# sanweiliti/LEMO

Measured on AMD Instinct MI355X. Metric: fitting-iterations/sec (T=120 frames), higher is better.
Workload: dtype f32; 1 GPU; opt_amass_temp.py temporal fit, one TotalCapture-shaped clip per GPU: B=119 frames (the T=120 clip), SMPL-X-shaped synthetic model V=10475, VPoser decode, smoothness encoder 245x134, marker+contact+prior losses, Adam; frames=119, vertices_per_frame=10475, sequences=1, conv_variant=9, parallelism=seq-shard x1 + 1 all_gather, hip_graph=True

## Files before the change

### lemo_amd/csrc/conv_turn_kernels.hip

```cpp
#include "conv_common.hpp"
#include "conv_f16.hpp"
#include "conv_pair.hpp"
#include "loss_device.hpp"

namespace lemo {

constexpr int TT_TH = 12, TT_TW = 12;
constexpr int TT_INW = TT_TW + 6, TT_INH = TT_TH + 4, TT_NIN = TT_INW * TT_INH;
constexpr int TT_ZW = TT_TW + 4, TT_ZH = TT_TH + 2, TT_NZ = TT_ZW * TT_ZH;
constexpr int TT_DW = TT_TW + 2, TT_DH = TT_TH + 2, TT_ND = TT_DW * TT_DH;
constexpr int TT_DP = 20, TT_NDP = TT_DP * TT_DH;
constexpr int TT_NOUT = TT_TH * TT_TW;
constexpr int TT_PL_IN = TT_NIN * 16, TT_GRP_IN = 2 * TT_PL_IN;
constexpr int TT_PL_D = TT_NDP * 16, TT_GRP_D = 2 * TT_PL_D;
constexpr int TT_D_OFF = 8 * TT_GRP_IN;
constexpr int TT_WMAX_OFF = TT_D_OFF + 8 * TT_GRP_D;
constexpr int TT_SMEM = TT_WMAX_OFF + 4 * 8 * 4;
constexpr int TT_NSLOT = 5;
constexpr int TT_NITEM = 8 * TT_ND * 2, TT_KITEM = (TT_NITEM + 511) / 512;
constexpr int TT_FRAMES = 32;
static_assert(TT_ZW == 16 && TT_NZ == 7 * 32 && TT_INW == 18, "z N-tiles = 2 rows x 16 columns on the input grid of row pitch 18");
static_assert(4 * 2 * TT_NIN <= TT_NSLOT * 512 && TT_NOUT <= 5 * 32, "staging slots / output tiles");
static_assert(8 * 8 * 256 * 4 <= TT_D_OFF && 8 * 6 * 256 * 4 <= TT_D_OFF, "the K-half exchanges fit the dead input planes");
static_assert(8 * TT_NZ * 8 * 4 <= 8 * TT_GRP_D, "the fp32 z tile fits the (not yet written) dpre planes");

__constant__ unsigned short tt_pix[160] = {
    0,   1,   2,   3,   12,  13,  14,  15,  16,  17,  18,  19,  4,   5,   6,   7,   28,  29,  30,  31,  8,   9,   10,  11,
    20,  21,  22,  23,  32,  33,  34,  35,  24,  25,  26,  27,  48,  49,  50,  51,  52,  53,  54,  55,  36,  37,  38,  39,
    56,  57,  58,  59,  40,  41,  42,  43,  44,  45,  46,  47,  68,  69,  70,  71,  60,  61,  62,  63,  72,  73,  74,  75,
    84,  85,  86,  87,  64,  65,  66,  67,  88,  89,  90,  91,  76,  77,  78,  79,  80,  81,  82,  83,  92,  93,  94,  95,
    96,  97,  98,  99,  108, 109, 110, 111, 112, 113, 114, 115, 100, 101, 102, 103, 124, 125, 126, 127, 104, 105, 106, 107,
    116, 117, 118, 119, 128, 129, 130, 131, 120, 121, 122, 123, 256, 257, 258, 259, 260, 261, 262, 263, 132, 133, 134, 135,
    264, 265, 266, 267, 136, 137, 138, 139, 140, 141, 142, 143, 276, 277, 278, 279};

struct TurnArgs {
  const float* in;
  const uint4* wf;
  const uint4* wb;
  const float* bias;
  float* z;
  float* out;
  float* dpre;
  double* acc;
  float winvf, winvb, coef2;
  int H, W, ntx, ntiles;
  FrameLoss fl;
  int nfb;
  unsigned long long* dbg;
};

struct TurnZ { float4 v[8]; int po[2]; bool own[2]; };

template <int NT>
__device__ __forceinline__ void turn_forward(const TurnArgs& a, unsigned char* smem, float* smem_f, float* wmax, int y0, int x0, int g, int ch,
                                             int kh, int lane, int wave, uint4 (&ra)[CP_RA][2], float (&sc)[2], float (&sci)[2],
                                             float4 (&stB)[TT_NSLOT], const int (&dstB)[TT_NSLOT], TurnZ& zs) {
  const int j = lane & 31, h = lane >> 5, T0 = g ? 4 : 0;
  const int H = a.H, W = a.W, Wp = W + 2;
  int li[NT];
#pragma unroll
  for (int nt = 0; nt < NT; ++nt) li[nt] = (2 * (T0 + nt) + (j >> 4) + 1) * TT_INW + cp_lane_col(j) + 1;
  f32x16 acc[NT];
#pragma unroll
  for (int nt = 0; nt < NT; ++nt)
#pragma unroll
    for (int r = 0; r < 16; ++r) acc[nt][r] = 0.f;
  pair_kloop<NT, TT_GRP_IN, TT_PL_IN, TT_INW>(
      acc, ra, a.wf, smem, li, kh, ch, lane,
      [&](int cc, int tap) {
        if (cc != 0) return;
        if (tap == 0) {
          float m = 0.f;
#pragma unroll
          for (int k = 0; k < TT_NSLOT; ++k) m = absmax4(stB[k], m);
          m = wave_max(m);
          if (lane == 0) wmax[8 + wave] = m;
        }
        if (tap == 1) {
          __syncthreads();
          float mm = 0.f;
#pragma unroll
          for (int i = 0; i < 8; ++i) mm = fmaxf(mm, wmax[8 + i]);
          f16_scale_after(mm, sc[0], sc[1], sci[1]);
        }
#pragma unroll
        for (int k = 0; k < TT_NSLOT; ++k) {
          if (2 + (7 * k) / TT_NSLOT != tap) continue;
          uint2 s0, s1;
          split2x4(stB[k], sc[1], s0, s1);
          *reinterpret_cast<uint2*>(smem + 2 * TT_GRP_IN + dstB[k]) = s0;
          *reinterpret_cast<uint2*>(smem + 2 * TT_GRP_IN + dstB[k] + TT_PL_IN) = s1;
        }
      },
      [&](int cc) {
        __syncthreads();
        if (cc == 0) {
          const float f = sc[1] * sci[0];
#pragma unroll
          for (int nt = 0; nt < NT; ++nt)
#pragma unroll
            for (int r = 0; r < 16; ++r) acc[nt][r] *= f;
        }
      });
  {
    const float f = sci[1] * a.winvf;
#pragma unroll
    for (int nt = 0; nt < NT; ++nt)
#pragma unroll
      for (int r = 0; r < 16; ++r) acc[nt][r] *= f;
  }
  typedef PairSplit<NT> S;
  const int KHu = __builtin_amdgcn_readfirstlane(kh);
  int zp[2];
  bool inimg[2];
#pragma unroll
  for (int sl = 0; sl < 2; ++sl) {
    const int t = T0 + (sl == 0 ? KHu : (NT == 4 ? 2 + KHu : 2));
    const int zr = 2 * t + (j >> 4), zc = cp_lane_col(j);
    const int y = y0 - 1 + zr, x = x0 - 2 + zc;
    zp[sl] = zr * TT_ZW + zc;
    inimg[sl] = (unsigned)y < (unsigned)H && (unsigned)x < (unsigned)W;
    zs.own[sl] = inimg[sl] && zr >= 1 && zr <= TT_TH && zc >= 2 && zc <= TT_TW + 1;
    const int yc = y < 0 ? 0 : (y >= H ? H - 1 : y), xc = x < 0 ? 0 : (x >= W ? W - 1 : x);
    zs.po[sl] = (yc + 1) * Wp + (xc + 1);
  }
  float4 eo[S::NQ];
#pragma unroll
  for (int i = 0; i < S::NQ; ++i) {
    const int q = KHu ? S::keep_quad(1, i) : S::keep_quad(0, i);
    eo[i] = ld4(a.bias + ch * 32 + q * 8 + 4 * h);
  }
  float4 v[S::NQ];
  {
    float* red = smem_f + ((g * 2 + ch) * 2) * 2048 + lane * 4;
    if (KHu) pair_exchange<NT, 1>(acc, v, red + 2048, red);
    else pair_exchange<NT, 0>(acc, v, red, red + 2048);
  }
  float* zt = smem_f + TT_D_OFF / 4;
#pragma unroll
  for (int i = 0; i < S::NQ; ++i) {
    const int q = KHu ? S::keep_quad(1, i) : S::keep_quad(0, i);
    const int c0 = ch * 32 + q * 8 + 4 * h;
    float4 r = v[i];
    r.x = lrelu(r.x + eo[i].x); r.y = lrelu(r.y + eo[i].y); r.z = lrelu(r.z + eo[i].z); r.w = lrelu(r.w + eo[i].w);
    if (!(i < 4 ? inimg[0] : inimg[1])) r = make_float4(0.f, 0.f, 0.f, 0.f);
    st4(zt + ((c0 >> 3) * TT_NZ + (i < 4 ? zp[0] : zp[1])) * 8 + (c0 & 7), r);
    zs.v[i] = r;
  }
}

template <bool DBG, int NT>
__device__ __forceinline__ void turn_backward(const TurnArgs& a, unsigned char* smem, float* smem_f, int y0, int x0, int T0, int g, int ch,
                                              int kh, int lane, float smi, uint4 (&ra)[CP_RA][2]) {
  const int j = lane & 31, h = lane >> 5;
  const int Wp = a.W + 2, HWp = (a.H + 2) * Wp;
  int lo[NT], poff[NT];
  bool ok[NT];
#pragma unroll
  for (int nt = 0; nt < NT; ++nt) {
    const int e = tt_pix[(T0 + nt) * 32 + j], p = e & 255, oy = p / TT_TW, ox = p - oy * TT_TW;
    lo[nt] = (oy + 1) * TT_DP + ox + 1;
    const int y = y0 + oy, x = x0 + ox;
    ok[nt] = e < 256 && y < a.H && x < a.W;
    poff[nt] = ((y < a.H ? y : a.H - 1) + 1) * Wp + ((x < a.W ? x : a.W - 1) + 1);
  }
  f32x16 acc[NT];
#pragma unroll
  for (int nt = 0; nt < NT; ++nt)
#pragma unroll
    for (int r = 0; r < 16; ++r) acc[nt][r] = 0.f;
  pair_kloop<NT, TT_GRP_D, TT_PL_D, TT_DP>(acc, ra, a.wb, smem + TT_D_OFF, lo, kh, ch, lane, [](int, int) {}, [](int) {});
  {
    const float f = smi * a.winvb;
#pragma unroll
    for (int nt = 0; nt < NT; ++nt)
#pragma unroll
      for (int r = 0; r < 16; ++r) acc[nt][r] *= f;
  }
  typedef PairSplit<NT> S;
  const int KHu = __builtin_amdgcn_readfirstlane(kh);
  const int poA = KHu ? poff[1] : poff[0], poB = poff[NT - 1];
  const bool okA = KHu ? ok[1] : ok[0], okB = ok[NT - 1];
  float4 eo[S::NQ];
#pragma unroll
  for (int i = 0; i < S::NQ; ++i) {
    const int q = KHu ? S::keep_quad(1, i) : S::keep_quad(0, i);
    const int c0 = ch * 32 + q * 8 + 4 * h;
    eo[i] = ld4(a.in + ((size_t)(c0 >> 3) * HWp + (i < 4 ? poA : poB)) * 8 + (c0 & 7));
  }
  float* red = smem_f + ((g * 2 + ch) * 2) * 1536 + lane * 4;
  float4 v[S::NQ];
  if (KHu) pair_exchange<NT, 1>(acc, v, red + 1536, red);
  else pair_exchange<NT, 0>(acc, v, red, red + 1536);
#pragma unroll
  for (int i = 0; i < S::NQ; ++i) {
    const int q = KHu ? S::keep_quad(1, i) : S::keep_quad(0, i);
    const int c0 = ch * 32 + q * 8 + 4 * h;
    float4 r = v[i];
    r.x *= lrelu_grad_from_out(eo[i].x); r.y *= lrelu_grad_from_out(eo[i].y);
    r.z *= lrelu_grad_from_out(eo[i].z); r.w *= lrelu_grad_from_out(eo[i].w);
    if (i < 4 ? okA : okB) st4(a.out + ((size_t)(c0 >> 3) * HWp + (i < 4 ? poA : poB)) * 8 + (c0 & 7), r);
  }
}

template <bool DBG>
__global__ void __launch_bounds__(512)
conv3x3_turn_kernel(TurnArgs a) {
  const int tid = (int)threadIdx.x, lane = tid & 63, wave = tid >> 6;
  if ((int)blockIdx.x >= a.ntiles) {
    const int b = ((int)blockIdx.x - a.ntiles) * TT_FRAMES + wave * 4 + (lane >> 4);
    vertex_loss_row16(b, lane & 15, a.fl);
    return;
  }
  unsigned long long t_start = 0, t_pro = 0, t_z = 0, t_st = 0, t_pl = 0;
  if (DBG) t_start = __builtin_amdgcn_s_memtime();
  LEMO_DYN_SMEM(smem_f);
  unsigned char* smem = reinterpret_cast<unsigned char*>(smem_f);
  float* wmax = reinterpret_cast<float*>(smem + TT_WMAX_OFF);
  const int ng = wave & 1, ch = (wave >> 1) & 1, kh = wave >> 2;
  const int H = a.H, W = a.W, Wp = W + 2, HWp = (H + 2) * Wp;
  const unsigned in_gstride = (unsigned)HWp * 8u;
  int tile = (int)blockIdx.x;
  {
    const int q = a.ntiles >> 3, r = a.ntiles & 7, xcd = tile & 7, k = tile >> 3;
    tile = (xcd < r ? xcd * (q + 1) : r * (q + 1) + (xcd - r) * q) + k;
  }
  const int ty = tile / a.ntx, tx = tile - ty * a.ntx;
  const int y0 = ty * TT_TH, x0 = tx * TT_TW;
  const int g = __builtin_amdgcn_readfirstlane(ng ^ kh);

  uint4 ra[CP_RA][2];
  pair_preload_a(ra, a.wf, kh, ch, lane);

  unsigned offB[TT_NSLOT];
  int dstB[TT_NSLOT];
#pragma unroll
  for (int k = 0; k < TT_NSLOT; ++k) {
    int c0 = tid + k * 512;
    c0 = c0 < 4 * 2 * TT_NIN ? c0 : 4 * 2 * TT_NIN - 1;
    const int gg = c0 / (2 * TT_NIN), c = c0 - gg * (2 * TT_NIN);
    const int px = c >> 1, half = c & 1;
    const int r = px / TT_INW, col = px - r * TT_INW;
    int gy = y0 - 2 + r, gx = x0 - 3 + col;
    gy = (gy < -1 ? -1 : (gy > H ? H : gy)) + 1;
    gx = (gx < -1 ? -1 : (gx > W ? W : gx)) + 1;
    const int g0 = (gg >> 1) * 4 + (gg & 1);
    offB[k] = (unsigned)g0 * in_gstride + (unsigned)(gy * Wp + gx) * 8u + 4u * half;
    dstB[k] = g0 * TT_GRP_IN + px * 16 + 8 * half;
  }
  float4 stB[TT_NSLOT];
#pragma unroll
  for (int k = 0; k < TT_NSLOT; ++k) stB[k] = ld4(a.in + offB[k]);
  float sc[2] = {1.f, 1.f}, sci[2] = {1.f, 1.f};
  {
    float m = 0.f;
#pragma unroll
    for (int k = 0; k < TT_NSLOT; ++k) m = absmax4(stB[k], m);
    m = wave_max(m);
    if (lane == 0) wmax[wave] = m;
    __syncthreads();
    float mm = 0.f;
#pragma unroll
    for (int i = 0; i < 8; ++i) mm = fmaxf(mm, wmax[i]);
    f16_scale_for(mm, sc[0], sci[0]);
  }
#pragma unroll
  for (int k = 0; k < TT_NSLOT; ++k) {
    uint2 s0, s1;
    split2x4(stB[k], sc[0], s0, s1);
    *reinterpret_cast<uint2*>(smem + dstB[k]) = s0;
    *reinterpret_cast<uint2*>(smem + dstB[k] + TT_PL_IN) = s1;
  }
#pragma unroll
  for (int k = 0; k < TT_NSLOT; ++k) stB[k] = ld4(a.in + 2u * in_gstride + offB[k]);
  __syncthreads();
  if (DBG) t_pro = __builtin_amdgcn_s_memtime();

  TurnZ zs;
  if (g) turn_forward<3>(a, smem, smem_f, wmax, y0, x0, 1, ch, kh, lane, wave, ra, sc, sci, stB, dstB, zs);
  else turn_forward<4>(a, smem, smem_f, wmax, y0, x0, 0, ch, kh, lane, wave, ra, sc, sci, stB, dstB, zs);
  pair_preload_a(ra, a.wb, kh, ch, lane);
  __syncthreads();
  if (DBG) t_z = __builtin_amdgcn_s_memtime();

  const float* zt = smem_f + TT_D_OFF / 4;
  float4 dv[TT_KITEM];
  int dslot[TT_KITEM];
  float sq = 0.f, mloc = 0.f;
#pragma unroll
  for (int k = 0; k < TT_KITEM; ++k) {
    const int it = tid + k * 512, ic = it < TT_NITEM ? it : TT_NITEM - 1;
    const int half = ic & 1, rest = ic >> 1, gq = rest / TT_ND, dp = rest - gq * TT_ND;
    const int dr = dp / TT_DW, dc = dp - dr * TT_DW;
    const int y = y0 - 1 + dr, x = x0 - 1 + dc;
    const bool valid = it < TT_NITEM && (unsigned)y < (unsigned)H && (unsigned)x < (unsigned)W;
    const bool own = valid && dr >= 1 && dr <= TT_TH && dc >= 1 && dc <= TT_TW;
    const bool hasl = x >= 1, hasr = x <= W - 2;
    const float* zc = zt + (gq * TT_NZ + dr * TT_ZW + dc + 1) * 8 + 4 * half;
    const float4 c = ld4(zc), l = ld4(zc - 8), r = ld4(zc + 8);
    float4 gr = make_float4(0.f, 0.f, 0.f, 0.f);
    if (hasl) { gr.x += c.x - l.x; gr.y += c.y - l.y; gr.z += c.z - l.z; gr.w += c.w - l.w; }
    if (hasr) {
      const float d0 = r.x - c.x, d1 = r.y - c.y, d2 = r.z - c.z, d3 = r.w - c.w;
      if (own) sq += d0 * d0 + d1 * d1 + d2 * d2 + d3 * d3;
      gr.x -= d0; gr.y -= d1; gr.z -= d2; gr.w -= d3;
    }
    const float cf = a.coef2;
    float4 o = make_float4(cf * gr.x * lrelu_grad_from_out(c.x), cf * gr.y * lrelu_grad_from_out(c.y),
                           cf * gr.z * lrelu_grad_from_out(c.z), cf * gr.w * lrelu_grad_from_out(c.w));
    if (!valid) o = make_float4(0.f, 0.f, 0.f, 0.f);
    if (a.dpre && own) st4(a.dpre + ((size_t)gq * HWp + (y + 1) * Wp + (x + 1)) * 8 + 4 * half, o);
    dv[k] = o;
    dslot[k] = it < TT_NITEM ? gq * TT_GRP_D + (dr * TT_DP + dc) * 16 + 8 * half : -1;
    mloc = absmax4(o, mloc);
  }
  mloc = wave_max(mloc);
  sq = wave_sum(sq);
  if (lane == 0) { wmax[16 + wave] = mloc; wmax[24 + wave] = sq; }
  __syncthreads();
  if (DBG) t_st = __builtin_amdgcn_s_memtime();
  float sm, smi;
  {
    float mm = 0.f;
#pragma unroll
    for (int i = 0; i < 8; ++i) mm = fmaxf(mm, wmax[16 + i]);
    f16_scale_for(mm, sm, smi);
  }
  if (tid == 0 && a.acc) {
    const float s = ((((((wmax[24] + wmax[25]) + wmax[26]) + wmax[27]) + wmax[28]) + wmax[29]) + wmax[30]) + wmax[31];
    atomicAdd(a.acc + (blockIdx.x & 31) * 16, (double)s);
  }
#pragma unroll
  for (int k = 0; k < TT_KITEM; ++k) {
    if (dslot[k] < 0) continue;
    uint2 s0, s1;
    split2x4(dv[k], sm, s0, s1);
    *reinterpret_cast<uint2*>(smem + TT_D_OFF + dslot[k]) = s0;
    *reinterpret_cast<uint2*>(smem + TT_D_OFF + dslot[k] + TT_PL_D) = s1;
  }
  __syncthreads();
  if (DBG) t_pl = __builtin_amdgcn_s_memtime();

  if (g) turn_backward<DBG, 2>(a, smem, smem_f, y0, x0, 3, 1, ch, kh, lane, smi, ra);
  else turn_backward<DBG, 3>(a, smem, smem_f, y0, x0, 0, 0, ch, kh, lane, smi, ra);
  {
    const int KHu = __builtin_amdgcn_readfirstlane(kh), h = lane >> 5;
    const int nq = g ? PairSplit<3>::NQ : PairSplit<4>::NQ;
#pragma unroll
    for (int i = 0; i < 8; ++i) {
      if (i >= nq) continue;
      const int q = g ? (KHu ? PairSplit<3>::keep_quad(1, i) : PairSplit<3>::keep_quad(0, i))
                      : (KHu ? PairSplit<4>::keep_quad(1, i) : PairSplit<4>::keep_quad(0, i));
      const int c0 = ch * 32 + q * 8 + 4 * h;
      if (i < 4 ? zs.own[0] : zs.own[1]) st4(a.z + ((size_t)(c0 >> 3) * HWp + (i < 4 ? zs.po[0] : zs.po[1])) * 8 + (c0 & 7), zs.v[i]);
    }
  }
  if (DBG && lane == 0) {
    unsigned long long* r = a.dbg + ((size_t)blockIdx.x * 8 + wave) * 8;
    r[0] = __builtin_amdgcn_s_getreg(63492);
    r[1] = t_start; r[2] = t_pro; r[3] = t_z; r[4] = t_st; r[5] = t_pl; r[6] = __builtin_amdgcn_s_memtime(); r[7] = 0;
  }
}

int conv_turn_init() {
  static LdsOptinOnce once;
  return lds_optin(once, {{&conv3x3_turn_kernel<false>, TT_SMEM}, {&conv3x3_turn_kernel<true>, TT_SMEM}});
}

bool conv3x3_turn_supported(int H, int W) { return H >= 1 && W >= 2 && (long)H * W <= (1l << 24); }

int conv3x3_turn_tiles(int H, int W) { return ((W + TT_TW - 1) / TT_TW) * ((H + TT_TH - 1) / TT_TH); }

int conv3x3_turn_f16(const float* in, const void* wf, float winvf, const float* bias, const void* wb, float winvb, float* z, float* out,
                     double* acc, float coef2, int H, int W, float* dpre, const FrameLoss* fl, hipStream_t s, unsigned long long* dbg) {
  if (!conv3x3_turn_supported(H, W)) return LEMO_ERR_SHAPE;
  if (!in || !wf || !wb || !bias || !z || !out || !(winvf > 0.f) || !(winvb > 0.f)) return LEMO_ERR_ARG;
  if (fl && (fl->B < 1 || dbg)) return LEMO_ERR_ARG;
  if (int rc = conv_turn_init()) return rc;
  TurnArgs a{};
  a.in = in; a.wf = reinterpret_cast<const uint4*>(wf); a.wb = reinterpret_cast<const uint4*>(wb); a.bias = bias;
  a.z = z; a.out = out; a.dpre = dpre; a.acc = acc; a.winvf = winvf; a.winvb = winvb; a.coef2 = coef2; a.H = H; a.W = W;
  a.ntx = (W + TT_TW - 1) / TT_TW;
  a.ntiles = conv3x3_turn_tiles(H, W);
  if (fl) { a.fl = *fl; a.nfb = (fl->B + TT_FRAMES - 1) / TT_FRAMES; }
  a.dbg = dbg;
  if (dbg) hipLaunchKernelGGL((conv3x3_turn_kernel<true>), dim3(a.ntiles), dim3(512), TT_SMEM, s, a);
  else hipLaunchKernelGGL((conv3x3_turn_kernel<false>), dim3(a.ntiles + a.nfb), dim3(512), TT_SMEM, s, a);
  return (int)hipGetLastError();
}

}
```

Baseline: 3533 fitting-iterations/s.

## Compute smoothness gradient in registers via DPP row shifts instead of LDS z tile

The fp32 z tile is no longer written to shared memory and re-read by a separate thread-remapped pass. Each lane now computes the horizontal smoothness gradient and squared-difference sum from its own z registers, using DPP row shifts to get left and right neighbours, then writes the f16-split gradient directly into the dpre LDS planes. This removes one LDS round trip and one block barrier, and the dpre global store becomes a compile-time template option. The cost is more registers held across the backward pass (zs.d) and reliance on DPP row semantics for the 16-column neighbour layout at tile edges.

```diff
diff --git a/lemo_amd/csrc/conv_turn_kernels.hip b/lemo_amd/csrc/conv_turn_kernels.hip
--- a/lemo_amd/csrc/conv_turn_kernels.hip
+++ b/lemo_amd/csrc/conv_turn_kernels.hip
@@ -8,7 +8,7 @@
 constexpr int TT_TH = 12, TT_TW = 12;
 constexpr int TT_INW = TT_TW + 6, TT_INH = TT_TH + 4, TT_NIN = TT_INW * TT_INH;
 constexpr int TT_ZW = TT_TW + 4, TT_ZH = TT_TH + 2, TT_NZ = TT_ZW * TT_ZH;
-constexpr int TT_DW = TT_TW + 2, TT_DH = TT_TH + 2, TT_ND = TT_DW * TT_DH;
+constexpr int TT_DW = TT_TW + 2, TT_DH = TT_TH + 2;
 constexpr int TT_DP = 20, TT_NDP = TT_DP * TT_DH;
 constexpr int TT_NOUT = TT_TH * TT_TW;
 constexpr int TT_PL_IN = TT_NIN * 16, TT_GRP_IN = 2 * TT_PL_IN;
@@ -17,12 +17,10 @@
 constexpr int TT_WMAX_OFF = TT_D_OFF + 8 * TT_GRP_D;
 constexpr int TT_SMEM = TT_WMAX_OFF + 4 * 8 * 4;
 constexpr int TT_NSLOT = 5;
-constexpr int TT_NITEM = 8 * TT_ND * 2, TT_KITEM = (TT_NITEM + 511) / 512;
 constexpr int TT_FRAMES = 32;
 static_assert(TT_ZW == 16 && TT_NZ == 7 * 32 && TT_INW == 18, "z N-tiles = 2 rows x 16 columns on the input grid of row pitch 18");
 static_assert(4 * 2 * TT_NIN <= TT_NSLOT * 512 && TT_NOUT <= 5 * 32, "staging slots / output tiles");
 static_assert(8 * 8 * 256 * 4 <= TT_D_OFF && 8 * 6 * 256 * 4 <= TT_D_OFF, "the K-half exchanges fit the dead input planes");
-static_assert(8 * TT_NZ * 8 * 4 <= 8 * TT_GRP_D, "the fp32 z tile fits the (not yet written) dpre planes");
 
 __constant__ unsigned short tt_pix[160] = {
     0,   1,   2,   3,   12,  13,  14,  15,  16,  17,  18,  19,  4,   5,   6,   7,   28,  29,  30,  31,  8,   9,   10,  11,
@@ -49,7 +47,12 @@
   unsigned long long* dbg;
 };
 
-struct TurnZ { float4 v[8]; int po[2]; bool own[2]; };
+struct TurnZ { float4 v[8], d[8]; int po[2], ds[2]; bool own[2]; float mloc, sq; };
+
+template <int N>
+__device__ __forceinline__ float4 row_from_left(const float4& v) {
+  return make_float4(dpp_move<0x120 + N>(v.x), dpp_move<0x120 + N>(v.y), dpp_move<0x120 + N>(v.z), dpp_move<0x120 + N>(v.w));
+}
 
 template <int NT>
 __device__ __forceinline__ void turn_forward(const TurnArgs& a, unsigned char* smem, float* smem_f, float* wmax, int y0, int x0, int g, int ch,
@@ -111,15 +114,16 @@
   }
   typedef PairSplit<NT> S;
   const int KHu = __builtin_amdgcn_readfirstlane(kh);
-  int zp[2];
-  bool inimg[2];
+  bool inimg[2], hasl[2], hasr[2];
 #pragma unroll
   for (int sl = 0; sl < 2; ++sl) {
     const int t = T0 + (sl == 0 ? KHu : (NT == 4 ? 2 + KHu : 2));
     const int zr = 2 * t + (j >> 4), zc = cp_lane_col(j);
     const int y = y0 - 1 + zr, x = x0 - 2 + zc;
-    zp[sl] = zr * TT_ZW + zc;
     inimg[sl] = (unsigned)y < (unsigned)H && (unsigned)x < (unsigned)W;
+    hasl[sl] = x >= 1;
+    hasr[sl] = x <= W - 2;
+    zs.ds[sl] = zc >= 1 && zc <= TT_DW ? (zr * TT_DP + zc - 1) * 16 + 8 * h : -1;
     zs.own[sl] = inimg[sl] && zr >= 1 && zr <= TT_TH && zc >= 2 && zc <= TT_TW + 1;
     const int yc = y < 0 ? 0 : (y >= H ? H - 1 : y), xc = x < 0 ? 0 : (x >= W ? W - 1 : x);
     zs.po[sl] = (yc + 1) * Wp + (xc + 1);
@@ -136,17 +140,34 @@
     if (KHu) pair_exchange<NT, 1>(acc, v, red + 2048, red);
     else pair_exchange<NT, 0>(acc, v, red, red + 2048);
   }
-  float* zt = smem_f + TT_D_OFF / 4;
-#pragma unroll
-  for (int i = 0; i < S::NQ; ++i) {
-    const int q = KHu ? S::keep_quad(1, i) : S::keep_quad(0, i);
-    const int c0 = ch * 32 + q * 8 + 4 * h;
+#pragma unroll
+  for (int i = 0; i < S::NQ; ++i) {
     float4 r = v[i];
     r.x = lrelu(r.x + eo[i].x); r.y = lrelu(r.y + eo[i].y); r.z = lrelu(r.z + eo[i].z); r.w = lrelu(r.w + eo[i].w);
     if (!(i < 4 ? inimg[0] : inimg[1])) r = make_float4(0.f, 0.f, 0.f, 0.f);
-    st4(zt + ((c0 >> 3) * TT_NZ + (i < 4 ? zp[0] : zp[1])) * 8 + (c0 & 7), r);
     zs.v[i] = r;
   }
+  float sq = 0.f, mloc = 0.f;
+#pragma unroll
+  for (int i = 0; i < S::NQ; ++i) {
+    const int sl = i < 4 ? 0 : 1;
+    const float4 c = zs.v[i], l = row_from_left<1>(c), r = row_from_left<15>(c);
+    float4 gr = make_float4(0.f, 0.f, 0.f, 0.f);
+    if (hasl[sl]) { gr.x += c.x - l.x; gr.y += c.y - l.y; gr.z += c.z - l.z; gr.w += c.w - l.w; }
+    if (hasr[sl]) {
+      const float d0 = r.x - c.x, d1 = r.y - c.y, d2 = r.z - c.z, d3 = r.w - c.w;
+      if (zs.own[sl]) sq += d0 * d0 + d1 * d1 + d2 * d2 + d3 * d3;
+      gr.x -= d0; gr.y -= d1; gr.z -= d2; gr.w -= d3;
+    }
+    const float cf = a.coef2;
+    float4 o = make_float4(cf * gr.x * lrelu_grad_from_out(c.x), cf * gr.y * lrelu_grad_from_out(c.y),
+                           cf * gr.z * lrelu_grad_from_out(c.z), cf * gr.w * lrelu_grad_from_out(c.w));
+    if (!inimg[sl] || zs.ds[sl] < 0) o = make_float4(0.f, 0.f, 0.f, 0.f);
+    zs.d[i] = o;
+    mloc = absmax4(o, mloc);
+  }
+  zs.mloc = wave_max(mloc);
+  zs.sq = wave_sum(sq);
 }
 
 template <bool DBG, int NT>
@@ -203,7 +224,7 @@
   }
 }
 
-template <bool DBG>
+template <bool DBG, bool DPRE>
 __global__ void __launch_bounds__(512)
 conv3x3_turn_kernel(TurnArgs a) {
   const int tid = (int)threadIdx.x, lane = tid & 63, wave = tid >> 6;
@@ -212,7 +233,7 @@
     vertex_loss_row16(b, lane & 15, a.fl);
     return;
   }
-  unsigned long long t_start = 0, t_pro = 0, t_z = 0, t_st = 0, t_pl = 0;
+  unsigned long long t_start = 0, t_pro = 0, t_z = 0, t_pl = 0;
   if (DBG) t_start = __builtin_amdgcn_s_memtime();
   LEMO_DYN_SMEM(smem_f);
   unsigned char* smem = reinterpret_cast<unsigned char*>(smem_f);
@@ -280,45 +301,11 @@
   if (g) turn_forward<3>(a, smem, smem_f, wmax, y0, x0, 1, ch, kh, lane, wave, ra, sc, sci, stB, dstB, zs);
   else turn_forward<4>(a, smem, smem_f, wmax, y0, x0, 0, ch, kh, lane, wave, ra, sc, sci, stB, dstB, zs);
   pair_preload_a(ra, a.wb, kh, ch, lane);
+  if (lane == 0) { wmax[16 + wave] = zs.mloc; wmax[24 + wave] = zs.sq; }
+  if (DBG) t_z = __builtin_amdgcn_s_memtime();
   __syncthreads();
-  if (DBG) t_z = __builtin_amdgcn_s_memtime();
-
-  const float* zt = smem_f + TT_D_OFF / 4;
-  float4 dv[TT_KITEM];
-  int dslot[TT_KITEM];
-  float sq = 0.f, mloc = 0.f;
-#pragma unroll
-  for (int k = 0; k < TT_KITEM; ++k) {
-    const int it = tid + k * 512, ic = it < TT_NITEM ? it : TT_NITEM - 1;
-    const int half = ic & 1, rest = ic >> 1, gq = rest / TT_ND, dp = rest - gq * TT_ND;
-    const int dr = dp / TT_DW, dc = dp - dr * TT_DW;
-    const int y = y0 - 1 + dr, x = x0 - 1 + dc;
-    const bool valid = it < TT_NITEM && (unsigned)y < (unsigned)H && (unsigned)x < (unsigned)W;
-    const bool own = valid && dr >= 1 && dr <= TT_TH && dc >= 1 && dc <= TT_TW;
-    const bool hasl = x >= 1, hasr = x <= W - 2;
-    const float* zc = zt + (gq * TT_NZ + dr * TT_ZW + dc + 1) * 8 + 4 * half;
-    const float4 c = ld4(zc), l = ld4(zc - 8), r = ld4(zc + 8);
-    float4 gr = make_float4(0.f, 0.f, 0.f, 0.f);
-    if (hasl) { gr.x += c.x - l.x; gr.y += c.y - l.y; gr.z += c.z - l.z; gr.w += c.w - l.w; }
-    if (hasr) {
-      const float d0 = r.x - c.x, d1 = r.y - c.y, d2 = r.z - c.z, d3 = r.w - c.w;
-      if (own) sq += d0 * d0 + d1 * d1 + d2 * d2 + d3 * d3;
-      gr.x -= d0; gr.y -= d1; gr.z -= d2; gr.w -= d3;
-    }
-    const float cf = a.coef2;
-    float4 o = make_float4(cf * gr.x * lrelu_grad_from_out(c.x), cf * gr.y * lrelu_grad_from_out(c.y),
-                           cf * gr.z * lrelu_grad_from_out(c.z), cf * gr.w * lrelu_grad_from_out(c.w));
-    if (!valid) o = make_float4(0.f, 0.f, 0.f, 0.f);
-    if (a.dpre && own) st4(a.dpre + ((size_t)gq * HWp + (y + 1) * Wp + (x + 1)) * 8 + 4 * half, o);
-    dv[k] = o;
-    dslot[k] = it < TT_NITEM ? gq * TT_GRP_D + (dr * TT_DP + dc) * 16 + 8 * half : -1;
-    mloc = absmax4(o, mloc);
-  }
-  mloc = wave_max(mloc);
-  sq = wave_sum(sq);
-  if (lane == 0) { wmax[16 + wave] = mloc; wmax[24 + wave] = sq; }
-  __syncthreads();
-  if (DBG) t_st = __builtin_amdgcn_s_memtime();
+
+  const int KHu = __builtin_amdgcn_readfirstlane(kh), nq = g ? PairSplit<3>::NQ : PairSplit<4>::NQ;
   float sm, smi;
   {
     float mm = 0.f;
@@ -330,13 +317,19 @@
     const float s = ((((((wmax[24] + wmax[25]) + wmax[26]) + wmax[27]) + wmax[28]) + wmax[29]) + wmax[30]) + wmax[31];
     atomicAdd(a.acc + (blockIdx.x & 31) * 16, (double)s);
   }
-#pragma unroll
-  for (int k = 0; k < TT_KITEM; ++k) {
-    if (dslot[k] < 0) continue;
+  int cg[8];
+#pragma unroll
+  for (int i = 0; i < 8; ++i)
+    cg[i] = ch * 4 + (g ? (KHu ? PairSplit<3>::keep_quad(1, i) : PairSplit<3>::keep_quad(0, i))
+                        : (KHu ? PairSplit<4>::keep_quad(1, i) : PairSplit<4>::keep_quad(0, i)));
+#pragma unroll
+  for (int i = 0; i < 8; ++i) {
+    const int slot = i < 4 ? zs.ds[0] : zs.ds[1];
+    if (i >= nq || slot < 0) continue;
     uint2 s0, s1;
-    split2x4(dv[k], sm, s0, s1);
-    *reinterpret_cast<uint2*>(smem + TT_D_OFF + dslot[k]) = s0;
-    *reinterpret_cast<uint2*>(smem + TT_D_OFF + dslot[k] + TT_PL_D) = s1;
+    split2x4(zs.d[i], sm, s0, s1);
+    *reinterpret_cast<uint2*>(smem + TT_D_OFF + cg[i] * TT_GRP_D + slot) = s0;
+    *reinterpret_cast<uint2*>(smem + TT_D_OFF + cg[i] * TT_GRP_D + slot + TT_PL_D) = s1;
   }
   __syncthreads();
   if (DBG) t_pl = __builtin_amdgcn_s_memtime();
@@ -344,27 +337,26 @@
   if (g) turn_backward<DBG, 2>(a, smem, smem_f, y0, x0, 3, 1, ch, kh, lane, smi, ra);
   else turn_backward<DBG, 3>(a, smem, smem_f, y0, x0, 0, 0, ch, kh, lane, smi, ra);
   {
-    const int KHu = __builtin_amdgcn_readfirstlane(kh), h = lane >> 5;
-    const int nq = g ? PairSplit<3>::NQ : PairSplit<4>::NQ;
+    const int h = lane >> 5;
 #pragma unroll
     for (int i = 0; i < 8; ++i) {
-      if (i >= nq) continue;
-      const int q = g ? (KHu ? PairSplit<3>::keep_quad(1, i) : PairSplit<3>::keep_quad(0, i))
-                      : (KHu ? PairSplit<4>::keep_quad(1, i) : PairSplit<4>::keep_quad(0, i));
-      const int c0 = ch * 32 + q * 8 + 4 * h;
-      if (i < 4 ? zs.own[0] : zs.own[1]) st4(a.z + ((size_t)(c0 >> 3) * HWp + (i < 4 ? zs.po[0] : zs.po[1])) * 8 + (c0 & 7), zs.v[i]);
+      if (i >= nq || !(i < 4 ? zs.own[0] : zs.own[1])) continue;
+      const size_t o = ((size_t)cg[i] * HWp + (i < 4 ? zs.po[0] : zs.po[1])) * 8 + 4 * h;
+      st4(a.z + o, zs.v[i]);
+      if constexpr (DPRE) st4(a.dpre + o, zs.d[i]);
     }
   }
   if (DBG && lane == 0) {
     unsigned long long* r = a.dbg + ((size_t)blockIdx.x * 8 + wave) * 8;
     r[0] = __builtin_amdgcn_s_getreg(63492);
-    r[1] = t_start; r[2] = t_pro; r[3] = t_z; r[4] = t_st; r[5] = t_pl; r[6] = __builtin_amdgcn_s_memtime(); r[7] = 0;
+    r[1] = t_start; r[2] = t_pro; r[3] = t_z; r[4] = t_pl; r[5] = __builtin_amdgcn_s_memtime(); r[6] = 0; r[7] = 0;
   }
 }
 
 int conv_turn_init() {
   static LdsOptinOnce once;
-  return lds_optin(once, {{&conv3x3_turn_kernel<false>, TT_SMEM}, {&conv3x3_turn_kernel<true>, TT_SMEM}});
+  return lds_optin(once, {{&conv3x3_turn_kernel<false, false>, TT_SMEM}, {&conv3x3_turn_kernel<false, true>, TT_SMEM},
+                          {&conv3x3_turn_kernel<true, false>, TT_SMEM}, {&conv3x3_turn_kernel<true, true>, TT_SMEM}});
 }
 
 bool conv3x3_turn_supported(int H, int W) { return H >= 1 && W >= 2 && (long)H * W <= (1l << 24); }
@@ -384,8 +376,10 @@
   a.ntiles = conv3x3_turn_tiles(H, W);
   if (fl) { a.fl = *fl; a.nfb = (fl->B + TT_FRAMES - 1) / TT_FRAMES; }
   a.dbg = dbg;
-  if (dbg) hipLaunchKernelGGL((conv3x3_turn_kernel<true>), dim3(a.ntiles), dim3(512), TT_SMEM, s, a);
-  else hipLaunchKernelGGL((conv3x3_turn_kernel<false>), dim3(a.ntiles + a.nfb), dim3(512), TT_SMEM, s, a);
+  if (dbg && dpre) hipLaunchKernelGGL((conv3x3_turn_kernel<true, true>), dim3(a.ntiles), dim3(512), TT_SMEM, s, a);
+  else if (dbg) hipLaunchKernelGGL((conv3x3_turn_kernel<true, false>), dim3(a.ntiles), dim3(512), TT_SMEM, s, a);
+  else if (dpre) hipLaunchKernelGGL((conv3x3_turn_kernel<false, true>), dim3(a.ntiles + a.nfb), dim3(512), TT_SMEM, s, a);
+  else hipLaunchKernelGGL((conv3x3_turn_kernel<false, false>), dim3(a.ntiles + a.nfb), dim3(512), TT_SMEM, s, a);
   return (int)hipGetLastError();
 }
 
```

Result: no change. 3508 fitting-iterations/s (-0.7%).
